# double125/MADTP

Measured on AMD Instinct MI355X. Metric: images/sec forward, BLIP-base NLVR2 p=0.5 b64; pruned-token index match, higher is better.
Workload: dtype bf16

## Files before the change

### madtp_amd/csrc/prune.hip

```cpp
#include "common.h"
#include "internal.h"
#include <stdlib.h>
#include <string.h>
#include <atomic>
#include <chrono>
#include <mutex>
#include <vector>

#ifndef TRY
#define TRY(x) do { int _rc = (x); if (_rc) return _rc; } while (0)
#endif

namespace {

constexpr int MAXN = 1024;

__device__ __forceinline__ float block_sum(float v, float* red, int tid, int nwaves) {
    v = wave_sum(v);
    __syncthreads();
    if ((tid & 63) == 0) red[tid >> 6] = v;
    __syncthreads();
    float s = 0.f;
    for (int w = 0; w < nwaves; ++w) s += red[w];
    return s;
// ... 1515 lines not shown
                for (int kk = 0; kk < 2; ++kk) {
                    ah[kk] = pack_bf16x8(xa[t][kk][0], xa[t][kk][1]);
                    f32x4 r0, r1;
#pragma unroll
                    for (int e = 0; e < 4; ++e) {
                        r0[e] = xa[t][kk][0][e] - bf16_to_f32((bf16_t)ah[kk][e]);
                        r1[e] = xa[t][kk][1][e] - bf16_to_f32((bf16_t)ah[kk][4 + e]);
                    }
                    al[kk] = pack_bf16x8(r0, r1);
                }
#pragma unroll
                for (int kk = 0; kk < 2; ++kk) {
#pragma unroll
                    for (int j = 0; j < 4; ++j) acc[t][j] = __builtin_amdgcn_mfma_f32_16x16x32_bf16(bh[kk][j], ah[kk], acc[t][j], 0, 0, 0);
#pragma unroll
                    for (int j = 0; j < 4; ++j) acc[t][j] = __builtin_amdgcn_mfma_f32_16x16x32_bf16(bh[kk][j], al[kk], acc[t][j], 0, 0, 0);
#pragma unroll
                    for (int j = 0; j < 4; ++j) acc[t][j] = __builtin_amdgcn_mfma_f32_16x16x32_bf16(bl[kk][j], ah[kk], acc[t][j], 0, 0, 0);
                }
            }
        }
    }
#pragma unroll
    for (int t = 0; t < 2; ++t) {
        const int m = row0 + rg * 32 + t * 16 + l16;
        if (m < M) {
            float* o = out + (size_t)m * 128 + cw * 64 + 4 * g;
#pragma unroll
            for (int j = 0; j < 4; ++j) *(f32x4*)(o + 16 * j) = F16 ? acc[t][j] * out_scale : acc[t][j];
        }
    }
}

}

constexpr int SPLIT_MAX_B = 1024, SPLIT_MAX_G = 8;
static std::atomic<int> g_score_fast{0};
static bool score_fast() { return g_score_fast.load(std::memory_order_relaxed) != 0; }
extern "C" int madtp_set_score_fast(int on) { return g_score_fast.exchange(on ? 1 : 0, std::memory_order_relaxed); }

static bool split_enabled() {
    static int v = -1;
    if (v < 0) { const char* e = getenv("MADTP_TS_SPLIT"); v = e ? atoi(e) : 1; }
    return v != 0;
}

static int token_score_launch(const float* colsum_part, int n_row_tiles, const float* p0, const float* onorm,
                              const float* token_attn, int ldt, int ldb, int K, float temperature, float* score,
                              float* threshold, int32_t* count, int32_t* kmax, int B, int H, int N, int32_t* done_ctr,
                              int32_t* host_slot, int seq, void* stream, int32_t* tick = nullptr, float* part = nullptr) {
    if (!colsum_part || !p0 || !onorm || !token_attn || !score || !threshold || !count) return MADTP_E_BADARG;
    if (B <= 0 || H <= 0 || N < 2 || n_row_tiles <= 0 || !(temperature > 0.f)) return MADTP_E_BADARG;
    if (N - 1 > MAXN || K > 128 || K <= 0 || ldt < K) return MADTP_E_SHAPE;
    const size_t stage_bytes = (size_t)(N - 1) * K * sizeof(float);
    const bool staged = K % 4 == 0 && ldt % 4 == 0 && ldb % 4 == 0 && aligned16(token_attn) && stage_bytes <= 140 * 1024;
    if (staged) {
        if (score_fast()) {
            MADTP_ENSURE_MAX_LDS((token_score_kernel<true, true>), 140 * 1024);
            hipLaunchKernelGGL((token_score_kernel<true, true>), dim3(B), dim3(512), stage_bytes, (hipStream_t)stream, colsum_part,
                               n_row_tiles, p0, onorm, token_attn, ldt, ldb, K, temperature, score, threshold, count, kmax, H, N,
                               done_ctr, host_slot, seq);
        } else {
            MADTP_ENSURE_MAX_LDS(token_score_kernel<true>, 140 * 1024);
            hipLaunchKernelGGL(token_score_kernel<true>, dim3(B), dim3(512), stage_bytes, (hipStream_t)stream, colsum_part,
                               n_row_tiles, p0, onorm, token_attn, ldt, ldb, K, temperature, score, threshold, count, kmax, H, N,
                               done_ctr, host_slot, seq);
// ... 357 lines not shown
        if (split) {
            MADTP_ENSURE_MAX_LDS(query_att_ft_mma_kernel<true>, att_ft_mma_lds(true));
            hipLaunchKernelGGL(att_ft_stats_kernel<true>, dim3(a.nseg, B), dim3(256), 0, (hipStream_t)stream, a, K, inv_sqrt_sd, stats);
            hipLaunchKernelGGL(query_att_ft_mma_kernel<true>, dim3(dim / AB_COLS, B), dim3(256), att_ft_mma_lds(true),
                               (hipStream_t)stream, a, K, stats, out, inv_sqrt_sd, acc_flag, dim);
        } else {
            MADTP_ENSURE_MAX_LDS(query_att_ft_mma_kernel<false>, att_ft_mma_lds(false));
            hipLaunchKernelGGL(att_ft_stats_kernel<false>, dim3(a.nseg, B), dim3(256), 0, (hipStream_t)stream, a, K, inv_sqrt_sd, stats);
            hipLaunchKernelGGL(query_att_ft_mma_kernel<false>, dim3(dim / AB_COLS, B), dim3(256), att_ft_mma_lds(false),
                               (hipStream_t)stream, a, K, stats, out, inv_sqrt_sd, acc_flag, dim);
        }
        MADTP_LAUNCH_CHECK();
    }
    return 0;
}

extern "C" int madtp_vector_gather(const float* vectors, const int64_t* indices, float* out, int B, int L, int K, int D,
                                   void* stream) {
    if (!vectors || !indices || !out || B <= 0 || L <= 0 || K <= 0 || D <= 0) return MADTP_E_BADARG;
    if (D % 4) return MADTP_E_SHAPE;
    if (!aligned16(vectors) || !aligned16(out)) return MADTP_E_ALIGN;
    const int rows = B * K;
    hipLaunchKernelGGL(vector_gather_kernel, dim3((rows + 3) / 4), dim3(256), 0, (hipStream_t)stream, vectors, indices, out, L,
                       K, D / 4, rows);
    MADTP_LAUNCH_CHECK();
    return 0;
}

extern "C" int madtp_align_logits(const float* x, const void* sd_hi, const void* sd_lo, float* out, int M, int dim,
                                  int split_dtype, float out_scale, void* stream) {
    return madtp_i_align_logits(x, sd_hi, sd_lo, out, M, dim, split_dtype, out_scale, DevN{nullptr, 0, 0}, stream);
}
static int align_rows_auto(int M) { (void)M; return 64; }

int madtp_i_align_logits(const float* x, const void* sd_hi, const void* sd_lo, float* out, int M, int dim, int split_dtype,
                         float out_scale, DevN m_dev, void* stream) {
    if (!x || !sd_hi || !sd_lo || !out || M <= 0) return MADTP_E_BADARG;
    if (split_dtype != MADTP_BF16 && split_dtype != MADTP_F16S) return MADTP_E_DTYPE;
    if (dim % 128) return MADTP_E_SHAPE;
    if (!aligned16(x) || !aligned16(sd_hi) || !aligned16(sd_lo) || !aligned16(out)) return MADTP_E_ALIGN;
    constexpr int lds = AL_STAGES * 2 * AL_TILE;
    MADTP_ENSURE_MAX_LDS(align_logits_kernel<12>, lds);
    MADTP_ENSURE_MAX_LDS(align_logits_kernel<8>, lds);
    MADTP_ENSURE_MAX_LDS(align_logits_kernel<0>, lds);
    static int variant = -1;
    if (variant < 0) { const char* e = getenv("MADTP_ALIGN_KERNEL"); variant = e ? atoi(e) : 0; }
    static int rows_env = -1;
    if (rows_env < 0) { const char* e = getenv("MADTP_ALIGN_ROWS"); rows_env = e ? atoi(e) : 0; }
    const int rows_sel = rows_env == 64 || rows_env == 128 ? rows_env : align_rows_auto(M);
    if ((variant == 0 || split_dtype == MADTP_F16S) && rows_sel == 128 && !m_dev.p) {
        MADTP_ENSURE_MAX_LDS(align_ws2_kernel<false>, 2 * AW2_STAGE);
        MADTP_ENSURE_MAX_LDS(align_ws2_kernel<true>, 2 * AW2_STAGE);
        if (split_dtype == MADTP_F16S)
            hipLaunchKernelGGL(align_ws2_kernel<true>, dim3((M + 127) / 128), dim3(768), 2 * AW2_STAGE, (hipStream_t)stream, x,
                               (const char*)sd_hi, (const char*)sd_lo, out, M, dim, out_scale, m_dev);
        else
            hipLaunchKernelGGL(align_ws2_kernel<false>, dim3((M + 127) / 128), dim3(768), 2 * AW2_STAGE, (hipStream_t)stream, x,
                               (const char*)sd_hi, (const char*)sd_lo, out, M, dim, 1.f, m_dev);
        MADTP_LAUNCH_CHECK();
        return 0;
    }
    if (variant == 0 || split_dtype == MADTP_F16S) {
        MADTP_ENSURE_MAX_LDS(align_ws_kernel<false>, 3 * AW_STAGE);
        MADTP_ENSURE_MAX_LDS(align_ws_kernel<true>, 3 * AW_STAGE);
        if (split_dtype == MADTP_F16S)
            hipLaunchKernelGGL(align_ws_kernel<true>, dim3((M + 63) / 64), dim3(768), 3 * AW_STAGE, (hipStream_t)stream, x,
                               (const char*)sd_hi, (const char*)sd_lo, out, M, dim, out_scale, m_dev);
        else
            hipLaunchKernelGGL(align_ws_kernel<false>, dim3((M + 63) / 64), dim3(768), 3 * AW_STAGE, (hipStream_t)stream, x,
                               (const char*)sd_hi, (const char*)sd_lo, out, M, dim, 1.f, m_dev);
        MADTP_LAUNCH_CHECK();
        return 0;
    }
    auto kern = dim == 768 ? align_logits_kernel<12> : dim == 512 ? align_logits_kernel<8> : align_logits_kernel<0>;
    hipLaunchKernelGGL(kern, dim3((M + 63) / 64), dim3(256), lds, (hipStream_t)stream, x, (const char*)sd_hi,
                       (const char*)sd_lo, out, M, dim, m_dev);
    MADTP_LAUNCH_CHECK();
    return 0;
}
```

### madtp_amd/csrc/gemm_device.h

```cpp
#pragma once
#include "common.h"
#include <type_traits>

namespace {


constexpr int ROWB = 128;
constexpr int NTHREADS = 256;

struct GemmArgs {
    const char* A; const char* W; const float* bias; const float* residual; void* C;
    int M, N, K, lda, ldw, ldc, ldr, act, ntm, ntn, dbg, fast_epi, splitk, ngrp;
    const char* A2; const char* W2; const float* bias2; void* C2; int pair;
    float out_scale;
    float acc_scale;
    float acc_scale2;
    float* sk_ws; int* sk_tick; int sk;
    int desc;
    int* range_flag;
    const int32_t* m_dev; int m_mul;
};
struct F16P { unsigned short bits; };

struct F16S {};
// ... 137 lines not shown
            for (int i = 0; i < 2; ++i) {
                const int row = min(row_t + 32 * i + l32, g.M - 1);
#pragma unroll
                for (int jv = 0; jv < NJ; ++jv)
                    rv[i][jv] = *(const f32x4*)(g.residual + (size_t)row * g.ldr + (cok[jv] ? colv[jv] : 0));
            }
        }
        __builtin_amdgcn_sched_barrier(0);
        __builtin_amdgcn_s_waitcnt(0x0F70);
        __builtin_amdgcn_sched_barrier(0);
#pragma unroll
        for (int i = 0; i < 2; ++i)
#pragma unroll
            for (int jv = 0; jv < NJ; ++jv) {
                const int t0 = LP_OUT ? 8 * jv : 4 * jv;
                f32x4 v[NV];
#pragma unroll
                for (int u = 0; u < NV; ++u) {
#pragma unroll
                    for (int e = 0; e < 4; ++e)
                        v[u][e] = epi_act<FAST_ACT, ACT>(fmaf(acc[i][j][t0 + 4 * u + e], g.acc_scale, bv[jv][u][e])) * g.out_scale;
                    if constexpr (HAS_RES) v[u] += rv[i][jv];
                }
                const unsigned off = cok[jv] ? (unsigned)((32 * i + l32) * ldc + colv[jv]) * CSZ : 0x80000000u;
                u32x4 bits;
                if constexpr (OM == OM_BF16) bits = __builtin_bit_cast(u32x4, pack_bf16x8(v[0], v[1]));
                else if constexpr (OM == OM_F16) bits = __builtin_bit_cast(u32x4, pack_f16x8(v[0], v[1]));
                else bits = __builtin_bit_cast(u32x4, v[0]);
                __builtin_amdgcn_raw_buffer_store_b128(bits, crsrc, off, 0, 0);
            }
    }
}

template <int OM, int ACT, bool HAS_RES, int FM, int FN, int BM, int BN, bool FAST_ONLY = false, int RM = 1, int RN = 1>
__device__ __forceinline__ void epilogue(const GemmArgs& g, const f32x4 (&acc)[FM][FN], const f32x4 (&res)[RM][RN],
                                         int m0, int n0, int wr, int wc, int l16, int grp4, size_t c_off) {
    constexpr bool LP_OUT = OM != OM_F32;
    constexpr bool FAST_ACT = OM == OM_BF16 || OM == OM_F16;
    const bool c_bf16 = g.ldc < 0;
    const int ldc = c_bf16 ? -g.ldc : g.ldc;
            const int col_w = n0 + wc * (BN / 2);
            if (FAST_ONLY || g.fast_epi) {
                constexpr int NJ = LP_OUT ? FN / 2 : FN;
                constexpr int NV = LP_OUT ? 2 : 1;
                constexpr int CSZ = LP_OUT ? 2 : 4;
                constexpr bool RES_PREF = !LP_OUT && RM == FM;
                float range_mx = 0.f;
                const int row_t = m0 + wr * (BM / 2);
                const int rows_valid = max(min(g.M - row_t, BM / 2), 0);
                const unsigned long long cb = (unsigned long long)((char*)g.C + (c_off + (size_t)((g.dbg & 8) ? (row_t & 127) : row_t) * ldc) * CSZ);
                const unsigned cb_lo = __builtin_amdgcn_readfirstlane((unsigned)cb);
                const unsigned cb_hi = __builtin_amdgcn_readfirstlane((unsigned)(cb >> 32));
                const __amdgpu_buffer_rsrc_t crsrc = __builtin_amdgcn_make_buffer_rsrc(
                    (void*)(((unsigned long long)cb_hi << 32) | cb_lo), 0,
                    __builtin_amdgcn_readfirstlane(rows_valid * ldc * CSZ), 0x00020000);
                int colv[NJ];
                bool cok[NJ];
                f32x4 bv[NJ][NV];
#pragma unroll
                for (int jv = 0; jv < NJ; ++jv) {
                    colv[jv] = col_w + (LP_OUT ? 32 * jv + 8 * grp4 : 16 * jv + 4 * grp4);
                    cok[jv] = colv[jv] < g.N;
#pragma unroll
                    for (int u = 0; u < NV; ++u) bv[jv][u] = (f32x4){0.f, 0.f, 0.f, 0.f};
                }
                if (g.bias) {
#pragma unroll
                    for (int jv = 0; jv < NJ; ++jv)
#pragma unroll
                        for (int u = 0; u < NV; ++u) bv[jv][u] = *(const f32x4*)(g.bias + (cok[jv] ? colv[jv] : 0) + 4 * u);
                }
                constexpr bool RES_LOAD = HAS_RES && !RES_PREF;
                constexpr int IC = RES_LOAD ? (FM > 2 ? FM / 2 : FM) : FM;
                f32x4 rv[RES_LOAD ? IC : 1][RES_LOAD ? NJ : 1][NV];
#pragma unroll
                for (int i0 = 0; i0 < FM; i0 += IC) {
                    if constexpr (RES_LOAD) {
#pragma unroll
                        for (int ii = 0; ii < IC; ++ii) {
                            const int row = min(row_t + l16 + 16 * (i0 + ii), g.M - 1);
#pragma unroll
                            for (int jv = 0; jv < NJ; ++jv) {
                                const float* rp = g.residual + (size_t)row * g.ldr + (cok[jv] ? colv[jv] : 0);
#pragma unroll
                                for (int u = 0; u < NV; ++u) rv[ii][jv][u] = *(const f32x4*)(rp + 4 * u);
                            }
                        }
                    }
                    if (RES_LOAD || i0 == 0) {
                        __builtin_amdgcn_sched_barrier(0);
                        __builtin_amdgcn_s_waitcnt(0x0F70);
                        __builtin_amdgcn_sched_barrier(0);
                    }
#pragma unroll
                    for (int ii = 0; ii < IC; ++ii) {
                        const int i = i0 + ii;
#pragma unroll
                        for (int jv = 0; jv < NJ; ++jv) {
                            f32x4 v[NV];
#pragma unroll
                            for (int u = 0; u < NV; ++u) {
#pragma unroll
                                for (int e = 0; e < 4; ++e)
                                    v[u][e] = epi_act<FAST_ACT, ACT>(fmaf(acc[i][NV * jv + u][e], g.acc_scale, bv[jv][u][e])) * g.out_scale;
                                if constexpr (RES_PREF && HAS_RES) v[u] += res[i][jv];
                                if constexpr (RES_LOAD) v[u] += rv[ii][jv][u];
                            }
                            const unsigned off = cok[jv] ? (unsigned)((16 * i + l16) * ldc + colv[jv]) * CSZ : 0x80000000u;
                            u32x4 bits;
                            if constexpr (OM == OM_F16S) {
                                u32x4 lo_bits;
                                split_f16x8(v[0], v[1], bits, lo_bits);
                                __builtin_amdgcn_raw_buffer_store_b128(lo_bits, crsrc, cok[jv] ? off + (unsigned)g.N * 2u : off, 0, 0);
                                range_mx = f16_range_acc(f16_range_acc(range_mx, v[0]), v[1]);
                            } else if constexpr (OM == OM_BF16) bits = __builtin_bit_cast(u32x4, pack_bf16x8(v[0], v[1]));
                            else if constexpr (OM == OM_F16) {
                                bits = __builtin_bit_cast(u32x4, pack_f16x8(v[0], v[1]));
                            }
                            else bits = __builtin_bit_cast(u32x4, v[0]);
                            __builtin_amdgcn_raw_buffer_store_b128(bits, crsrc, off, 0, 0);
                        }
                    }
                }
                if constexpr (OM == OM_F16S) f16_range_raise(g.range_flag, !(range_mx < 65520.0f));
            } else if constexpr (!FAST_ONLY) {
#pragma unroll
                for (int j = 0; j < FN; ++j)
#pragma unroll
                    for (int r = 0; r < 4; ++r) {
                        const int col = col_w + wfrag_row<LP_OUT>(j, 4 * grp4 + r);
                        if (col >= g.N) continue;
                        const float bv = g.bias ? g.bias[col] : 0.0f;
#pragma unroll
                        for (int i = 0; i < FM; ++i) {
                            const int row = m0 + wr * (BM / 2) + i * 16 + l16;
                            if (row >= g.M) continue;
                            float v = epi_act<FAST_ACT, ACT>(fmaf(acc[i][j][r], g.acc_scale, bv)) * g.out_scale;
                            if (g.residual) v += g.residual[(size_t)row * g.ldr + col];
                            const size_t ci = c_off + (size_t)row * ldc + col;
                            if constexpr (OM == OM_F16S) {
                                const _Float16 h = (_Float16)v;
                                ((_Float16*)g.C)[ci] = h;
                                ((_Float16*)g.C)[ci + g.N] = (_Float16)((v - (float)h) * F16S_LO_SCALE);
                                f16_range_raise(g.range_flag, f16_range_bad(v));
                            } else if constexpr (OM == OM_F16) {
                                ((_Float16*)g.C)[ci] = (_Float16)v;
                                f16_range_raise(g.range_flag, f16_range_bad(v));
                            } else if (c_bf16) ((bf16_t*)g.C)[ci] = f32_to_bf16(v);
                            else ((float*)g.C)[ci] = v;
                        }
                    }
            }
}

// ... 2 lines not shown
```

### madtp_amd/csrc/gemm_pp.hip

```cpp
#include "gemm_device.h"
#include <stdlib.h>

template <int OM, int MODE, int FA = 4, int ABL = 0, bool SPLITK = false>
__global__ __launch_bounds__(512, 2) void gemm_pp_kernel(GemmArgs g) {
    static_assert(FA == 4 || FA == 3, "256- or 192-row tiles");
    constexpr bool X3 = MODE == 2, F16 = MODE != 0;
    constexpr bool LP_OUT = OM != OM_F32;
    constexpr int BM = 64 * FA, BN = 256, HT = 128 * ROWB;
    extern __shared__ __attribute__((aligned(16))) char smem[];

    const int xcd = blockIdx.x & 7, lb = blockIdx.x >> 3, gl = gridDim.x >> 3;
    const int S = SPLITK ? g.splitk : 1;
    int t0, nslots;
    xcd_tiles(g.ntm * g.ntn * S, xcd, t0, nslots);
    if (lb >= nslots) return;

    const int tid = threadIdx.x, lane = tid & 63;
    const int wave = __builtin_amdgcn_readfirstlane(tid >> 6);
    const int wr = wave >> 2, wc = wave & 3;
    const int nkp = g.K / 64;
    const int nks = __builtin_amdgcn_readfirstlane(nkp / S);

    constexpr int WJ1 = (wfrag_row<LP_OUT>(1, 0) - wfrag_row<LP_OUT>(0, 0)) * ROWB;
    const char* ab[2][2];
    const char* wb[2][2];
    auto frag_bases = [&]() {
        int ln = lane;
        asm volatile("" : "+v"(ln));
        const int l16 = ln & 15, grp4 = ln >> 4;
        const int ra0 = wr * 64 + l16, rw0 = wc * 32 + wfrag_row<LP_OUT>(0, l16);
        const int a_rd = ra0 * ROWB + ((grp4 ^ (l16 & 7)) << 4);
        const int w_rd = rw0 * ROWB + ((grp4 ^ swz_key<LP_OUT>(rw0)) << 4);
        ab[0][0] = smem + a_rd; ab[0][1] = smem + (a_rd ^ 64); ab[1][0] = smem + 65536 + a_rd; ab[1][1] = smem + 65536 + (a_rd ^ 64);
        wb[0][0] = smem + w_rd; wb[0][1] = smem + (w_rd ^ 64); wb[1][0] = smem + 65536 + w_rd; wb[1][1] = smem + 65536 + (w_rd ^ 64);
    };
    frag_bases();

    const int npad = ((g.N + 127) / 128) * 128;
    const __amdgpu_buffer_rsrc_t rs_a = __builtin_amdgcn_make_buffer_rsrc((void*)g.A, 0, (unsigned)((size_t)g.M * g.lda * 2), 0x00020000);
    const __amdgpu_buffer_rsrc_t rs_w = __builtin_amdgcn_make_buffer_rsrc((void*)g.W, 0, (unsigned)((size_t)npad * g.ldw * 2), 0x00020000);
    unsigned va[2][2], vw[2][2];
    int is_slot = lb, is_koff = 0, is_kend = nkp * ROWB;
// ... 47 lines not shown
            is_koff += ROWB;                                                                   \
            if (is_koff == is_kend) { is_slot += gl; tile_offsets(); unit_krange(); }          \
        }                                                                                      \
        is_offa = is_koff + ((X3 && is_s == 2) ? plane_b : 0);                                 \
        is_offw = is_koff + ((X3 && is_s == 0) ? plane_b : 0);                                 \
    } while (0)

    f32x4 acc[2 * FA][4];
    bf16x8 a0[FA][2], a1[FA][2], b0[2][2], b1[2][2];
    const f32x4 zero4 = (f32x4){0.f, 0.f, 0.f, 0.f};
    f32x4 res[1][1];
#define PP_FENCE() __builtin_amdgcn_sched_barrier(0)
#define PP_READ_A(R, P, IDX)                                                                   \
    if (!(ABL & 4) || !steady)                                                                 \
    _Pragma("unroll") for (int i = 0; i < FA; ++i) {                                           \
        R[i][0] = *(const bf16x8*)(ab[P][0] + (IDX) * HT + i * 16 * ROWB);                     \
        R[i][1] = *(const bf16x8*)(ab[P][1] + (IDX) * HT + i * 16 * ROWB);                     \
    }
#define PP_READ_W(R, P, IDX)                                                                   \
    if (!(ABL & 4) || !steady)                                                                 \
    _Pragma("unroll") for (int j = 0; j < 2; ++j) {                                            \
        R[j][0] = *(const bf16x8*)(wb[P][0] + (IDX) * HT + j * WJ1);                           \
        R[j][1] = *(const bf16x8*)(wb[P][1] + (IDX) * HT + j * WJ1);                           \
    }
#define PP_MFMA(RA, RW, SA, SB)                                                                \
    if (!(ABL & 2))                                                                            \
    _Pragma("unroll") for (int ks = 0; ks < 2; ++ks)                                           \
        _Pragma("unroll") for (int i = 0; i < FA; ++i)                                         \
            _Pragma("unroll") for (int j = 0; j < 2; ++j)                                      \
                acc[(SA) * FA + i][(SB) * 2 + j] = mfma_16x16x32<F16>(RW[j][ks], RA[i][ks], acc[(SA) * FA + i][(SB) * 2 + j]);
#define PP_SCALE_W(R, ON)                                                                      \
    if constexpr (X3 && (ON))                                                                  \
    _Pragma("unroll") for (int j = 0; j < 2; ++j) { R[j][0] = x3_scale_lo(R[j][0]); R[j][1] = x3_scale_lo(R[j][1]); }
#define PP_PHASE(READS, ISSUE, PRE, MFMAS)                                                     \
    {                                                                                          \
        READS                                                                                  \
        PP_FENCE();                                                                            \
        if constexpr (!(ABL & 8)) { ISSUE }                                                    \
        PP_FENCE();                                                                            \
        wait_vmcnt<(ABL & 8) ? 8 : 10>();                                                      \
        PP_FENCE();                                                                            \
        __builtin_amdgcn_s_barrier();                                                          \
        PP_FENCE();                                                                            \
        if constexpr ((ABL & 8) != 0) { ISSUE }                                                \
        PP_FENCE();                                                                            \
        __builtin_amdgcn_s_waitcnt(0xC07F);                                    \
        PP_FENCE();                                                                            \
        PRE                                                                                    \
        PP_FENCE();                                                                            \
        if constexpr (!(ABL & 16)) __builtin_amdgcn_s_setprio(1);                              \
        MFMAS                                                                                  \
        if constexpr (!(ABL & 16)) __builtin_amdgcn_s_setprio(0);                              \
        PP_FENCE();                                                                            \
        __builtin_amdgcn_s_barrier();                                                          \
        PP_FENCE();                                                                            \
    }
#define PP_SLAB(P, SC)                                                                                                              \
    PP_PHASE(PP_READ_A(a0, P, 1), PP_ISSUE_W(vw[1], 4 * ((P) ^ 1) + 3); PP_NEXT_SLAB();, PP_SCALE_W(b0, SC), PP_MFMA(a0, b0, 0, 0))   \
    PP_PHASE(PP_READ_A(a1, P, 2), PP_ISSUE_W(vw[0], 4 * (P) + 0);, , PP_MFMA(a1, b0, 1, 0))                                          \
    PP_PHASE(PP_READ_W(b1, P, 3), PP_ISSUE_A(va[0], 4 * (P) + 1);, PP_SCALE_W(b1, SC), PP_MFMA(a1, b1, 1, 1))                        \
    PP_PHASE(PP_READ_W(b0, (P) ^ 1, 0), PP_ISSUE_A(va[1], 4 * (P) + 2);, , PP_MFMA(a0, b1, 0, 1))

    PP_ISSUE_W(vw[0], 0); PP_ISSUE_A(va[0], 1); PP_ISSUE_A(va[1], 2); PP_ISSUE_W(vw[1], 3);
    PP_NEXT_SLAB();
    PP_ISSUE_W(vw[0], 4); PP_ISSUE_A(va[0], 5); PP_ISSUE_A(va[1], 6);
    PP_FENCE();
    wait_vmcnt<10>();
    __builtin_amdgcn_s_barrier();
    PP_FENCE();

    for (int slot = lb; slot < nslots; slot += gl) {
        if (wr == 1) __builtin_amdgcn_s_barrier();
        PP_FENCE();
        if (slot != lb) { frag_bases(); tile_offsets(); }
        PP_READ_W(b0, 0, 0)
        PP_FENCE();
        __builtin_amdgcn_s_waitcnt(0xC07F);
        PP_FENCE();
#pragma unroll
        for (int i = 0; i < 2 * FA; ++i)
#pragma unroll
            for (int j = 0; j < 4; ++j) acc[i][j] = zero4;
        for (int kt = 0; kt < nks; kt += 2) {
            if constexpr (X3) {
                PP_SLAB(0, false)
                PP_SLAB(1, false)
                PP_SLAB(0, true)
                PP_SLAB(1, false)
                PP_SLAB(0, false)
                PP_SLAB(1, true)
            } else {
                PP_SLAB(0, false)
                PP_SLAB(1, false)
            }
            steady = true;
        }
        if (wr == 0) __builtin_amdgcn_s_barrier();
        PP_FENCE();
        int ctm, ctn;
        const int cu = t0 + slot, ct = S > 1 ? __builtin_amdgcn_readfirstlane(cu / S) : cu;
        tile_mn(g, ct, ctm, ctn);
        const size_t c_off = S > 1 ? (size_t)(cu - ct * S) * g.M * (size_t)(g.ldc < 0 ? -g.ldc : g.ldc) : 0;
        const int m0 = ctm * BM, n0 = ctn * BN + (wc >> 1) * 128;
        int lne = lane;
        asm volatile("" : "+v"(lne));
        const int l16e = lne & 15, grp4e = lne >> 4;
#define EPI(ACT)                                                                                                  \
    if constexpr (LP_OUT) {                                                                                       \
        epilogue<OM, ACT, false, 2 * FA, 4, BM, 128>(g, acc, res, m0, n0, wr, wc & 1, l16e, grp4e, c_off);             \
    } else {                                                                                                      \
        if (g.residual) epilogue<OM, ACT, true, 2 * FA, 4, BM, 128>(g, acc, res, m0, n0, wr, wc & 1, l16e, grp4e, c_off); \
        else epilogue<OM, ACT, false, 2 * FA, 4, BM, 128>(g, acc, res, m0, n0, wr, wc & 1, l16e, grp4e, c_off);        \
    }
        switch (g.act) {
            case MADTP_ACT_GELU_ERF: EPI(MADTP_ACT_GELU_ERF) break;
            case MADTP_ACT_QUICK_GELU: EPI(MADTP_ACT_QUICK_GELU) break;
            case MADTP_ACT_RELU: EPI(MADTP_ACT_RELU) break;
            default: EPI(MADTP_ACT_NONE) break;
        }
#undef EPI
    }
    wait_vmcnt<0>();
#undef PP_SLAB
#undef PP_PHASE
#undef PP_SCALE_W
#undef PP_ISSUE_A
#undef PP_ISSUE_W
#undef PP_MFMA
#undef PP_READ_W
#undef PP_READ_A
#undef PP_FENCE
#undef PP_NEXT_SLAB
#undef PP_ISSUE
}

__attribute__((visibility("hidden"))) int madtp_gemm_pp_launch(const void* args, int om, int mode, int rows, int grid, void* stream) {
    const GemmArgs& g = *(const GemmArgs*)args;
    hipStream_t s = (hipStream_t)stream;
    const size_t lds = (size_t)8 * 128 * ROWB;
    static int abl = -1;
    if (abl < 0) { const char* e = getenv("MADTP_PP_ABLATE"); abl = e ? atoi(e) : 0; }
#define PP_LAUNCH(OM_, MODE_, FA_, ABL_)                                                                        \
    do {                                                                                                        \
        MADTP_ENSURE_MAX_LDS((gemm_pp_kernel<OM_, MODE_, FA_, ABL_>), lds);                                      \
        hipLaunchKernelGGL((gemm_pp_kernel<OM_, MODE_, FA_, ABL_>), dim3(grid), dim3(512), lds, s, g);           \
    } while (0)
#define PP_ROWS(OM_, MODE_)                                                                                     \
    do { if (rows == 192) PP_LAUNCH(OM_, MODE_, 3, 0); else PP_LAUNCH(OM_, MODE_, 4, 0); } while (0)
    if (rows != 256 && rows != 192) return MADTP_E_BADARG;
    if (g.splitk > 1) {
        if (mode != 2 || om != OM_F32 || rows != 256 || g.bias || g.residual || g.act != MADTP_ACT_NONE) return MADTP_E_DTYPE;
        MADTP_ENSURE_MAX_LDS((gemm_pp_kernel<OM_F32, 2, 4, 0, true>), lds);
        hipLaunchKernelGGL((gemm_pp_kernel<OM_F32, 2, 4, 0, true>), dim3(grid), dim3(512), lds, s, g);
        return 0;
    }
    if (mode == 2) {
        if (om == OM_F16S) PP_ROWS(OM_F16S, 2); else if (om == OM_F32) PP_ROWS(OM_F32, 2); else return MADTP_E_DTYPE;
    } else if (mode == 1) {
        if (om == OM_F16) PP_ROWS(OM_F16, 1); else if (om == OM_F32) PP_ROWS(OM_F32, 1); else return MADTP_E_DTYPE;
    } else if (om == OM_BF16) {
        switch (rows == 256 ? abl : 0) {
#ifdef MADTP_PP_ABLATIONS
            case 1: PP_LAUNCH(OM_BF16, 0, 4, 1); break;
            case 2: PP_LAUNCH(OM_BF16, 0, 4, 2); break;
            case 3: PP_LAUNCH(OM_BF16, 0, 4, 3); break;
            case 4: PP_LAUNCH(OM_BF16, 0, 4, 4); break;
            case 5: PP_LAUNCH(OM_BF16, 0, 4, 5); break;
            case 6: PP_LAUNCH(OM_BF16, 0, 4, 6); break;
            case 8: PP_LAUNCH(OM_BF16, 0, 4, 8); break;
            case 16: PP_LAUNCH(OM_BF16, 0, 4, 16); break;
#endif
            default: PP_ROWS(OM_BF16, 0); break;
        }
    } else if (om == OM_F32) {
        PP_ROWS(OM_F32, 0);
    } else {
        return MADTP_E_DTYPE;
    }
#undef PP_ROWS
#undef PP_LAUNCH
    return 0;
}
```

Baseline: 26390.

## Add warp-specialized register-prefetch align-logits kernel with column split for small M

```diff
diff --git a/madtp_amd/csrc/prune.hip b/madtp_amd/csrc/prune.hip
--- a/madtp_amd/csrc/prune.hip
+++ b/madtp_amd/csrc/prune.hip
@@ -1571,6 +1571,147 @@
     }
 }
 
+constexpr int AR_STAGES = 4, AR_AHEAD = 3;
+template <bool F16, int NK, int COLS>
+__global__ __launch_bounds__(COLS * 6, 1) void align_rx_kernel(const float* __restrict__ x, const char* __restrict__ sd_hi,
+                                                               const char* __restrict__ sd_lo, float* __restrict__ out, int M,
+                                                               float out_scale, DevN m_dev) {
+    extern __shared__ __attribute__((aligned(16))) char smem[];
+    M = devn(m_dev, M);
+    if ((int)blockIdx.x * 64 >= M) return;
+    static_assert(COLS == 128 || COLS == 64, "column tile");
+    constexpr int dim = NK * 64;
+    constexpr int TILE = COLS * AL_ROWB, STAGE = 2 * TILE;
+    constexpr int NCONS = COLS / 16, PER = 8;
+    const int tid = threadIdx.x, lane = tid & 63;
+    const int wave = __builtin_amdgcn_readfirstlane(tid >> 6);
+    const int row0 = blockIdx.x * 64;
+    const int cb = COLS == 128 ? 0 : blockIdx.y * 64;
+    if (wave >= NCONS) {
+        const int lw = wave - NCONS;
+        const char* srcp[PER];
+#pragma unroll
+        for (int q = 0; q < PER; ++q) {
+            const int idx = lw * PER + q;
+            const int grp = idx % (COLS / 8), r = grp * 8 + (lane >> 3);
+            const char* base = idx < COLS / 8 ? sd_hi : sd_lo;
+            srcp[q] = base + (size_t)(cb + r) * dim * 2 + (((lane & 7) ^ (r & 7)) << 4);
+        }
+        auto issue = [&](int kt) {
+            char* st = smem + (kt % AR_STAGES) * STAGE + lw * PER * 1024;
+#pragma unroll
+            for (int q = 0; q < PER; ++q)
+                __builtin_amdgcn_global_load_lds(GLOBAL_PTR(srcp[q] + kt * AL_ROWB), LDS_PTR(st + q * 1024), 16, 0, 0);
+        };
+#pragma unroll
+        for (int kt = 0; kt < AR_AHEAD && kt < NK; ++kt) issue(kt);
+        for (int kt = 0; kt < NK; ++kt) {
+            if (kt + 2 < NK) asm volatile("s_waitcnt vmcnt(16)" ::: "memory");
+            else if (kt + 1 < NK) asm volatile("s_waitcnt vmcnt(8)" ::: "memory");
+            else asm volatile("s_waitcnt vmcnt(0)" ::: "memory");
+            __builtin_amdgcn_s_barrier();
+            if (kt + AR_AHEAD < NK) issue(kt + AR_AHEAD);
+        }
+        return;
+    }
+    const int l16 = lane & 15, g = lane >> 4;
+    const int rw = wave & 3, cw = wave >> 2;
+    const int xr = rw * 16 + l16;
+    const int cl = cw * 64;
+    int row = row0 + xr;
+    row = row < M ? row : M - 1;
+    const float* xp = x + (size_t)row * dim + g * 8;
+    f32x4 xq[AR_AHEAD][2][2];
+    auto load_x = [&](int kt, f32x4 (&d)[2][2]) {
+#pragma unroll
+        for (int kk = 0; kk < 2; ++kk) {
+            const float* p = xp + kt * 64 + kk * 32;
+            d[kk][0] = *(const f32x4*)p;
+            d[kk][1] = *(const f32x4*)(p + 4);
+        }
+    };
+#pragma unroll
+    for (int kt = 0; kt < AR_AHEAD && kt < NK; ++kt) load_x(kt, xq[kt]);
+    f32x4 acc[4];
+#pragma unroll
+    for (int j = 0; j < 4; ++j) acc[j] = (f32x4){0.f, 0.f, 0.f, 0.f};
+#pragma unroll
+    for (int kt = 0; kt < NK; ++kt) {
+        f32x4 (&xa)[2][2] = xq[kt % AR_AHEAD];
+        bf16x8 ah[2], al[2];
+        if constexpr (F16) {
+#pragma unroll
+            for (int kk = 0; kk < 2; ++kk) {
+                u32x4 p0, p1;
+                split_f16x8(xa[kk][0], xa[kk][1], p0, p1);
+                ah[kk] = __builtin_bit_cast(bf16x8, p0);
+                al[kk] = __builtin_bit_cast(bf16x8, p1);
+            }
+        } else {
+#pragma unroll
+            for (int kk = 0; kk < 2; ++kk) {
+                ah[kk] = pack_bf16x8(xa[kk][0], xa[kk][1]);
+                f32x4 r0, r1;
+#pragma unroll
+                for (int e = 0; e < 4; ++e) {
+                    r0[e] = xa[kk][0][e] - bf16_to_f32((bf16_t)ah[kk][e]);
+                    r1[e] = xa[kk][1][e] - bf16_to_f32((bf16_t)ah[kk][4 + e]);
+                }
+                al[kk] = pack_bf16x8(r0, r1);
+            }
+        }
+        __builtin_amdgcn_sched_barrier(0);
+        if (kt + AR_AHEAD < NK) load_x(kt + AR_AHEAD, xa);
+        const char* sh = smem + (kt % AR_STAGES) * STAGE;
+        const char* sl = sh + TILE;
+        __builtin_amdgcn_s_barrier();
+        bf16x8 bh[2][4], bl[2][4];
+#pragma unroll
+        for (int kk = 0; kk < 2; ++kk)
+#pragma unroll
+            for (int j = 0; j < 4; ++j) {
+                const int rb = cl + j * 16 + l16;
+                const int off = rb * AL_ROWB + (((kk * 4 + g) ^ (rb & 7)) << 4);
+                bh[kk][j] = *(const bf16x8*)(sh + off);
+                bl[kk][j] = *(const bf16x8*)(sl + off);
+            }
+        if constexpr (F16) {
+#pragma unroll
+            for (int kk = 0; kk < 2; ++kk) {
+#pragma unroll
+                for (int j = 0; j < 4; ++j)
+                    acc[j] = __builtin_amdgcn_mfma_f32_16x16x32_f16(__builtin_bit_cast(f16x8, bl[kk][j]), __builtin_bit_cast(f16x8, ah[kk]), acc[j], 0, 0, 0);
+#pragma unroll
+                for (int j = 0; j < 4; ++j)
+                    acc[j] = __builtin_amdgcn_mfma_f32_16x16x32_f16(__builtin_bit_cast(f16x8, bh[kk][j]), __builtin_bit_cast(f16x8, ah[kk]), acc[j], 0, 0, 0);
+#pragma unroll
+                for (int j = 0; j < 4; ++j) {
+                    const f16x8 q2 = __builtin_bit_cast(f16x8, bh[kk][j]) * (_Float16)(1.0f / F16S_LO_SCALE);
+                    acc[j] = __builtin_amdgcn_mfma_f32_16x16x32_f16(q2, __builtin_bit_cast(f16x8, al[kk]), acc[j], 0, 0, 0);
+                }
+            }
+        } else {
+#pragma unroll
+            for (int kk = 0; kk < 2; ++kk) {
+#pragma unroll
+                for (int j = 0; j < 4; ++j) acc[j] = __builtin_amdgcn_mfma_f32_16x16x32_bf16(bh[kk][j], ah[kk], acc[j], 0, 0, 0);
+#pragma unroll
+                for (int j = 0; j < 4; ++j) acc[j] = __builtin_amdgcn_mfma_f32_16x16x32_bf16(bh[kk][j], al[kk], acc[j], 0, 0, 0);
+#pragma unroll
+                for (int j = 0; j < 4; ++j) acc[j] = __builtin_amdgcn_mfma_f32_16x16x32_bf16(bl[kk][j], ah[kk], acc[j], 0, 0, 0);
+            }
+        }
+        asm volatile("s_waitcnt lgkmcnt(0)" ::: "memory");
+        __builtin_amdgcn_sched_barrier(0);
+    }
+    const int m = row0 + xr;
+    if (m < M) {
+        float* o = out + (size_t)m * 128 + cb + cl + 4 * g;
+#pragma unroll
+        for (int j = 0; j < 4; ++j) *(f32x4*)(o + 16 * j) = F16 ? acc[j] * out_scale : acc[j];
+    }
+}
+
 }
 
 constexpr int SPLIT_MAX_B = 1024, SPLIT_MAX_G = 8;
@@ -1994,6 +2135,7 @@
     return madtp_i_align_logits(x, sd_hi, sd_lo, out, M, dim, split_dtype, out_scale, DevN{nullptr, 0, 0}, stream);
 }
 static int align_rows_auto(int M) { (void)M; return 64; }
+static int align_variant_auto(int M) { return M <= 1280 ? 2 : 0; }
 
 int madtp_i_align_logits(const float* x, const void* sd_hi, const void* sd_lo, float* out, int M, int dim, int split_dtype,
                          float out_scale, DevN m_dev, void* stream) {
@@ -2010,6 +2152,31 @@
     static int rows_env = -1;
     if (rows_env < 0) { const char* e = getenv("MADTP_ALIGN_ROWS"); rows_env = e ? atoi(e) : 0; }
     const int rows_sel = rows_env == 64 || rows_env == 128 ? rows_env : align_rows_auto(M);
+    static int rx_env = -2;
+    if (rx_env == -2) { const char* e = getenv("MADTP_ALIGN_VARIANT"); rx_env = e ? atoi(e) : -1; }
+    const bool rx_ok = dim == 768 || dim == 512;
+    int rx = rx_env >= 0 ? rx_env : (rows_env == 64 || rows_env == 128 || variant != 0) ? 0 : align_variant_auto(M);
+    if (rx < 0 || rx > 2 || !rx_ok) rx = 0;
+    if (rx) {
+#define ALIGN_RX_LAUNCH(F16_, NK_, COLS_, SCALE_)                                                                              \
+    do {                                                                                                                       \
+        constexpr int lds_rx = AR_STAGES * 2 * COLS_ * AL_ROWB;                                                                \
+        MADTP_ENSURE_MAX_LDS((align_rx_kernel<F16_, NK_, COLS_>), lds_rx);                                                     \
+        hipLaunchKernelGGL((align_rx_kernel<F16_, NK_, COLS_>), dim3((M + 63) / 64, 128 / COLS_), dim3(COLS_ * 6), lds_rx,     \
+                           (hipStream_t)stream, x, (const char*)sd_hi, (const char*)sd_lo, out, M, SCALE_, m_dev);             \
+    } while (0)
+        const bool f16 = split_dtype == MADTP_F16S;
+        if (rx == 1) {
+            if (dim == 768) { if (f16) ALIGN_RX_LAUNCH(true, 12, 128, out_scale); else ALIGN_RX_LAUNCH(false, 12, 128, 1.f); }
+            else { if (f16) ALIGN_RX_LAUNCH(true, 8, 128, out_scale); else ALIGN_RX_LAUNCH(false, 8, 128, 1.f); }
+        } else {
+            if (dim == 768) { if (f16) ALIGN_RX_LAUNCH(true, 12, 64, out_scale); else ALIGN_RX_LAUNCH(false, 12, 64, 1.f); }
+            else { if (f16) ALIGN_RX_LAUNCH(true, 8, 64, out_scale); else ALIGN_RX_LAUNCH(false, 8, 64, 1.f); }
+        }
+#undef ALIGN_RX_LAUNCH
+        MADTP_LAUNCH_CHECK();
+        return 0;
+    }
     if ((variant == 0 || split_dtype == MADTP_F16S) && rows_sel == 128 && !m_dev.p) {
         MADTP_ENSURE_MAX_LDS(align_ws2_kernel<false>, 2 * AW2_STAGE);
         MADTP_ENSURE_MAX_LDS(align_ws2_kernel<true>, 2 * AW2_STAGE);
```

New measurement: 26150. About the same (-0.9%).

## Prefetch bias into LDS and double-buffer residual loads in GEMM epilogue

Applied to the files above, without the earlier changes.

```diff
diff --git a/madtp_amd/csrc/gemm_device.h b/madtp_amd/csrc/gemm_device.h
--- a/madtp_amd/csrc/gemm_device.h
+++ b/madtp_amd/csrc/gemm_device.h
@@ -193,9 +193,9 @@
     }
 }
 
-template <int OM, int ACT, bool HAS_RES, int FM, int FN, int BM, int BN, bool FAST_ONLY = false, int RM = 1, int RN = 1>
+template <int OM, int ACT, bool HAS_RES, int FM, int FN, int BM, int BN, bool FAST_ONLY = false, int RM = 1, int RN = 1, int BND = 0>
 __device__ __forceinline__ void epilogue(const GemmArgs& g, const f32x4 (&acc)[FM][FN], const f32x4 (&res)[RM][RN],
-                                         int m0, int n0, int wr, int wc, int l16, int grp4, size_t c_off) {
+                                         int m0, int n0, int wr, int wc, int l16, int grp4, size_t c_off, const char* sbias = nullptr) {
     constexpr bool LP_OUT = OM != OM_F32;
     constexpr bool FAST_ACT = OM == OM_BF16 || OM == OM_F16;
     const bool c_bf16 = g.ldc < 0;
@@ -208,7 +208,7 @@
                 constexpr bool RES_PREF = !LP_OUT && RM == FM;
                 float range_mx = 0.f;
                 const int row_t = m0 + wr * (BM / 2);
-                const int rows_valid = max(min(g.M - row_t, BM / 2), 0);
+                const int rows_valid = max(min(BND ? __builtin_amdgcn_readfirstlane(g.M - row_t) : g.M - row_t, BM / 2), 0);
                 const unsigned long long cb = (unsigned long long)((char*)g.C + (c_off + (size_t)((g.dbg & 8) ? (row_t & 127) : row_t) * ldc) * CSZ);
                 const unsigned cb_lo = __builtin_amdgcn_readfirstlane((unsigned)cb);
                 const unsigned cb_hi = __builtin_amdgcn_readfirstlane((unsigned)(cb >> 32));
@@ -229,29 +229,49 @@
 #pragma unroll
                     for (int jv = 0; jv < NJ; ++jv)
 #pragma unroll
-                        for (int u = 0; u < NV; ++u) bv[jv][u] = *(const f32x4*)(g.bias + (cok[jv] ? colv[jv] : 0) + 4 * u);
+                        for (int u = 0; u < NV; ++u) {
+                            if constexpr (BND & 1) bv[jv][u] = *(const f32x4*)(sbias + (colv[jv] - n0 + 4 * u) * 4);
+                            else bv[jv][u] = *(const f32x4*)(g.bias + (cok[jv] ? colv[jv] : 0) + 4 * u);
+                        }
                 }
                 constexpr bool RES_LOAD = HAS_RES && !RES_PREF;
-                constexpr int IC = RES_LOAD ? (FM > 2 ? FM / 2 : FM) : FM;
-                f32x4 rv[RES_LOAD ? IC : 1][RES_LOAD ? NJ : 1][NV];
+                constexpr bool RES_PIPE = RES_LOAD && (BND & 2) != 0 && !LP_OUT && (FM % 2) == 0 && FM > 2;
+                constexpr int IC = RES_PIPE ? 2 : (RES_LOAD ? (FM > 2 ? FM / 2 : FM) : FM);
+                [[maybe_unused]] constexpr int PER = IC * NJ * NV;
+                f32x4 rv[RES_PIPE ? 2 : 1][RES_LOAD ? IC : 1][RES_LOAD ? NJ : 1][NV];
+                auto res_load = [&](int b, int i0) {
+#pragma unroll
+                    for (int ii = 0; ii < IC; ++ii) {
+                        const int row = min(row_t + l16 + 16 * (i0 + ii), g.M - 1);
+#pragma unroll
+                        for (int jv = 0; jv < NJ; ++jv) {
+                            const float* rp = g.residual + (size_t)row * g.ldr + (cok[jv] ? colv[jv] : 0);
+#pragma unroll
+                            for (int u = 0; u < NV; ++u) rv[b][ii][jv][u] = *(const f32x4*)(rp + 4 * u);
+                        }
+                    }
+                };
+                if constexpr (RES_PIPE) {
+                    res_load(0, 0);
+                    __builtin_amdgcn_sched_barrier(0);
+                    res_load(1, IC);
+                }
 #pragma unroll
                 for (int i0 = 0; i0 < FM; i0 += IC) {
-                    if constexpr (RES_LOAD) {
-#pragma unroll
-                        for (int ii = 0; ii < IC; ++ii) {
-                            const int row = min(row_t + l16 + 16 * (i0 + ii), g.M - 1);
-#pragma unroll
-                            for (int jv = 0; jv < NJ; ++jv) {
-                                const float* rp = g.residual + (size_t)row * g.ldr + (cok[jv] ? colv[jv] : 0);
-#pragma unroll
-                                for (int u = 0; u < NV; ++u) rv[ii][jv][u] = *(const f32x4*)(rp + 4 * u);
-                            }
-                        }
-                    }
-                    if (RES_LOAD || i0 == 0) {
+                    const int rb = RES_PIPE ? (i0 / IC) & 1 : 0;
+                    if constexpr (RES_PIPE) {
                         __builtin_amdgcn_sched_barrier(0);
-                        __builtin_amdgcn_s_waitcnt(0x0F70);
+                        if (i0 == 0) wait_vmcnt<PER>();
+                        else if (i0 + IC < FM) wait_vmcnt<2 * PER>();
+                        else wait_vmcnt<PER>();
                         __builtin_amdgcn_sched_barrier(0);
+                    } else {
+                        if constexpr (RES_LOAD) res_load(0, i0);
+                        if (RES_LOAD || (i0 == 0 && !(BND & 1))) {
+                            __builtin_amdgcn_sched_barrier(0);
+                            __builtin_amdgcn_s_waitcnt(0x0F70);
+                            __builtin_amdgcn_sched_barrier(0);
+                        }
                     }
 #pragma unroll
                     for (int ii = 0; ii < IC; ++ii) {
@@ -265,7 +285,7 @@
                                 for (int e = 0; e < 4; ++e)
                                     v[u][e] = epi_act<FAST_ACT, ACT>(fmaf(acc[i][NV * jv + u][e], g.acc_scale, bv[jv][u][e])) * g.out_scale;
                                 if constexpr (RES_PREF && HAS_RES) v[u] += res[i][jv];
-                                if constexpr (RES_LOAD) v[u] += rv[ii][jv][u];
+                                if constexpr (RES_LOAD) v[u] += rv[rb][ii][jv][u];
                             }
                             const unsigned off = cok[jv] ? (unsigned)((16 * i + l16) * ldc + colv[jv]) * CSZ : 0x80000000u;
                             u32x4 bits;
@@ -281,6 +301,10 @@
                             else bits = __builtin_bit_cast(u32x4, v[0]);
                             __builtin_amdgcn_raw_buffer_store_b128(bits, crsrc, off, 0, 0);
                         }
+                    }
+                    if constexpr (RES_PIPE) {
+                        __builtin_amdgcn_sched_barrier(0);
+                        if (i0 + 2 * IC < FM) res_load(rb, i0 + 2 * IC);
                     }
                 }
                 if constexpr (OM == OM_F16S) f16_range_raise(g.range_flag, !(range_mx < 65520.0f));
diff --git a/madtp_amd/csrc/gemm_pp.hip b/madtp_amd/csrc/gemm_pp.hip
--- a/madtp_amd/csrc/gemm_pp.hip
+++ b/madtp_amd/csrc/gemm_pp.hip
@@ -1,13 +1,32 @@
 #include "gemm_device.h"
 #include <stdlib.h>
 
-template <int OM, int MODE, int FA = 4, int ABL = 0, bool SPLITK = false>
+#ifndef MADTP_PP_BOUNDARY
+#if defined(MADTP_PP_TIMING) && MADTP_PP_TIMING == 1
+#define MADTP_PP_BOUNDARY 0
+#else
+#define MADTP_PP_BOUNDARY 3
+#endif
+#endif
+#ifdef MADTP_PP_TIMING
+__device__ long long g_pp_dbg[32];
+__device__ __forceinline__ long long pp_now() {
+    __builtin_amdgcn_sched_barrier(0);
+    __builtin_amdgcn_s_waitcnt(0xC07F);
+    const long long t = wall_clock64();
+    __builtin_amdgcn_sched_barrier(0);
+    return t;
+}
+#endif
+template <int OM, int MODE, int FA = 4, int ABL = 0, bool SPLITK = false, bool GEN = false>
 __global__ __launch_bounds__(512, 2) void gemm_pp_kernel(GemmArgs g) {
     static_assert(FA == 4 || FA == 3, "256- or 192-row tiles");
     constexpr bool X3 = MODE == 2, F16 = MODE != 0;
     constexpr bool LP_OUT = OM != OM_F32;
     constexpr int BM = 64 * FA, BN = 256, HT = 128 * ROWB;
+    constexpr int BND = SPLITK ? 0 : (MADTP_PP_BOUNDARY);
     extern __shared__ __attribute__((aligned(16))) char smem[];
+    char* const sbias = smem + 8 * HT;
 
     const int xcd = blockIdx.x & 7, lb = blockIdx.x >> 3, gl = gridDim.x >> 3;
     const int S = SPLITK ? g.splitk : 1;
@@ -121,13 +140,23 @@
 #define PP_SCALE_W(R, ON)                                                                      \
     if constexpr (X3 && (ON))                                                                  \
     _Pragma("unroll") for (int j = 0; j < 2; ++j) { R[j][0] = x3_scale_lo(R[j][0]); R[j][1] = x3_scale_lo(R[j][1]); }
-#define PP_PHASE(READS, ISSUE, PRE, MFMAS)                                                     \
+#ifdef MADTP_PP_TIMING
+#define PP_WAIT(PH)                                                                            \
+    if (ts_first) {                                                                            \
+        const long long t__ = pp_now();                                                        \
+        wait_vmcnt<10>();                                                                      \
+        ts_ph##PH += pp_now() - t__;                                                           \
+    } else wait_vmcnt<10>()
+#else
+#define PP_WAIT(PH) wait_vmcnt<(ABL & 8) ? 8 : 10>()
+#endif
+#define PP_PHASE(PH, READS, ISSUE, PRE, MFMAS)                                                 \
     {                                                                                          \
         READS                                                                                  \
         PP_FENCE();                                                                            \
         if constexpr (!(ABL & 8)) { ISSUE }                                                    \
         PP_FENCE();                                                                            \
-        wait_vmcnt<(ABL & 8) ? 8 : 10>();                                                      \
+        PP_WAIT(PH);                                                                           \
         PP_FENCE();                                                                            \
         __builtin_amdgcn_s_barrier();                                                          \
         PP_FENCE();                                                                            \
@@ -145,10 +174,10 @@
         PP_FENCE();                                                                            \
     }
 #define PP_SLAB(P, SC)                                                                                                              \
-    PP_PHASE(PP_READ_A(a0, P, 1), PP_ISSUE_W(vw[1], 4 * ((P) ^ 1) + 3); PP_NEXT_SLAB();, PP_SCALE_W(b0, SC), PP_MFMA(a0, b0, 0, 0))   \
-    PP_PHASE(PP_READ_A(a1, P, 2), PP_ISSUE_W(vw[0], 4 * (P) + 0);, , PP_MFMA(a1, b0, 1, 0))                                          \
-    PP_PHASE(PP_READ_W(b1, P, 3), PP_ISSUE_A(va[0], 4 * (P) + 1);, PP_SCALE_W(b1, SC), PP_MFMA(a1, b1, 1, 1))                        \
-    PP_PHASE(PP_READ_W(b0, (P) ^ 1, 0), PP_ISSUE_A(va[1], 4 * (P) + 2);, , PP_MFMA(a0, b1, 0, 1))
+    PP_PHASE(0, PP_READ_A(a0, P, 1), PP_ISSUE_W(vw[1], 4 * ((P) ^ 1) + 3); PP_NEXT_SLAB();, PP_SCALE_W(b0, SC), PP_MFMA(a0, b0, 0, 0))   \
+    PP_PHASE(1, PP_READ_A(a1, P, 2), PP_ISSUE_W(vw[0], 4 * (P) + 0);, , PP_MFMA(a1, b0, 1, 0))                                          \
+    PP_PHASE(2, PP_READ_W(b1, P, 3), PP_ISSUE_A(va[0], 4 * (P) + 1);, PP_SCALE_W(b1, SC), PP_MFMA(a1, b1, 1, 1))                        \
+    PP_PHASE(3, PP_READ_W(b0, (P) ^ 1, 0), PP_ISSUE_A(va[1], 4 * (P) + 2);, , PP_MFMA(a0, b1, 0, 1))
 
     PP_ISSUE_W(vw[0], 0); PP_ISSUE_A(va[0], 1); PP_ISSUE_A(va[1], 2); PP_ISSUE_W(vw[1], 3);
     PP_NEXT_SLAB();
@@ -158,9 +187,27 @@
     __builtin_amdgcn_s_barrier();
     PP_FENCE();
 
+#ifdef MADTP_PP_TIMING
+    const bool ts_on = blockIdx.x == 0 && wc == 0;
+    long long ts_main = 0, ts_entry = 0, ts_epi = 0, ts_ph0 = 0, ts_ph1 = 0, ts_ph2 = 0, ts_ph3 = 0, ts_tiles = 0, ts_after = 0;
+    const long long ts_start = ts_on ? pp_now() : 0;
+    bool ts_first = false;
+#endif
     for (int slot = lb; slot < nslots; slot += gl) {
         if (wr == 1) __builtin_amdgcn_s_barrier();
         PP_FENCE();
+        if constexpr ((BND & 1) != 0) {
+            if (wave == 4 && g.bias && g.fast_epi) {
+                int btm, btn;
+                tile_mn(g, t0 + slot, btm, btn);
+                const __amdgpu_buffer_rsrc_t rs_b = __builtin_amdgcn_make_buffer_rsrc((void*)g.bias, 0, (unsigned)g.N * 4u, 0x00020000);
+                __builtin_amdgcn_raw_ptr_buffer_load_lds(rs_b, LDS_PTR(sbias), 16, (unsigned)lane * 16u, btn * (BN * 4), 0, 0);
+            }
+            PP_FENCE();
+        }
+#ifdef MADTP_PP_TIMING
+        const long long ts_t0 = ts_on ? pp_now() : 0;
+#endif
         if (slot != lb) { frag_bases(); tile_offsets(); }
         PP_READ_W(b0, 0, 0)
         PP_FENCE();
@@ -171,8 +218,15 @@
 #pragma unroll
             for (int j = 0; j < 4; ++j) acc[i][j] = zero4;
         for (int kt = 0; kt < nks; kt += 2) {
+#ifdef MADTP_PP_TIMING
+            ts_first = ts_on && kt == 0 && slot != lb;
+#define PP_TS_FIRST_OFF() ts_first = false;
+#else
+#define PP_TS_FIRST_OFF()
+#endif
             if constexpr (X3) {
                 PP_SLAB(0, false)
+                PP_TS_FIRST_OFF()
                 PP_SLAB(1, false)
                 PP_SLAB(0, true)
                 PP_SLAB(1, false)
@@ -180,36 +234,58 @@
                 PP_SLAB(1, true)
             } else {
                 PP_SLAB(0, false)
+                PP_TS_FIRST_OFF()
                 PP_SLAB(1, false)
             }
             steady = true;
         }
         if (wr == 0) __builtin_amdgcn_s_barrier();
         PP_FENCE();
+#ifdef MADTP_PP_TIMING
+        long long ts_t1 = 0;
+        if (ts_on) {
+            ts_t1 = pp_now();
+            ts_main += ts_t1 - ts_t0;
+            if constexpr (!(BND & 1)) { wait_vmcnt<0>(); const long long t__ = pp_now(); ts_entry += t__ - ts_t1; ts_t1 = t__; }
+        }
+#endif
         int ctm, ctn;
         const int cu = t0 + slot, ct = S > 1 ? __builtin_amdgcn_readfirstlane(cu / S) : cu;
         tile_mn(g, ct, ctm, ctn);
         const size_t c_off = S > 1 ? (size_t)(cu - ct * S) * g.M * (size_t)(g.ldc < 0 ? -g.ldc : g.ldc) : 0;
         const int m0 = ctm * BM, n0 = ctn * BN + (wc >> 1) * 128;
-        int lne = lane;
-        asm volatile("" : "+v"(lne));
-        const int l16e = lne & 15, grp4e = lne >> 4;
+        const char* const sbw = sbias + (wc >> 1) * 512;
 #define EPI(ACT)                                                                                                  \
+    int lne = lane;                                                                                               \
+    asm volatile("" : "+v"(lne));                                                                                 \
+    const int l16e = lne & 15, grp4e = lne >> 4;                                                                  \
     if constexpr (LP_OUT) {                                                                                       \
-        epilogue<OM, ACT, false, 2 * FA, 4, BM, 128>(g, acc, res, m0, n0, wr, wc & 1, l16e, grp4e, c_off);             \
+        epilogue<OM, ACT, false, 2 * FA, 4, BM, 128, !GEN, 1, 1, BND>(g, acc, res, m0, n0, wr, wc & 1, l16e, grp4e, c_off, sbw);             \
     } else {                                                                                                      \
-        if (g.residual) epilogue<OM, ACT, true, 2 * FA, 4, BM, 128>(g, acc, res, m0, n0, wr, wc & 1, l16e, grp4e, c_off); \
-        else epilogue<OM, ACT, false, 2 * FA, 4, BM, 128>(g, acc, res, m0, n0, wr, wc & 1, l16e, grp4e, c_off);        \
+        if (g.residual) epilogue<OM, ACT, true, 2 * FA, 4, BM, 128, !GEN, 1, 1, BND>(g, acc, res, m0, n0, wr, wc & 1, l16e, grp4e, c_off, sbw); \
+        else epilogue<OM, ACT, false, 2 * FA, 4, BM, 128, !GEN, 1, 1, BND>(g, acc, res, m0, n0, wr, wc & 1, l16e, grp4e, c_off, sbw);        \
     }
         switch (g.act) {
-            case MADTP_ACT_GELU_ERF: EPI(MADTP_ACT_GELU_ERF) break;
-            case MADTP_ACT_QUICK_GELU: EPI(MADTP_ACT_QUICK_GELU) break;
-            case MADTP_ACT_RELU: EPI(MADTP_ACT_RELU) break;
-            default: EPI(MADTP_ACT_NONE) break;
+            case MADTP_ACT_GELU_ERF: { EPI(MADTP_ACT_GELU_ERF) } break;
+            case MADTP_ACT_QUICK_GELU: { EPI(MADTP_ACT_QUICK_GELU) } break;
+            case MADTP_ACT_RELU: { EPI(MADTP_ACT_RELU) } break;
+            default: { EPI(MADTP_ACT_NONE) } break;
         }
 #undef EPI
+#ifdef MADTP_PP_TIMING
+        if (ts_on) { ts_epi += pp_now() - ts_t1; ts_tiles += 1; ts_after += slot != lb; }
+#endif
     }
     wait_vmcnt<0>();
+#ifdef MADTP_PP_TIMING
+    if (ts_on && lane == 0) {
+        long long* d = g_pp_dbg + 16 * wr;
+        d[0] = ts_main; d[1] = ts_entry; d[2] = ts_epi; d[3] = ts_ph0; d[4] = ts_ph1; d[5] = ts_ph2; d[6] = ts_ph3;
+        d[7] = ts_tiles; d[8] = pp_now() - ts_start; d[9] = ts_after;
+    }
+#endif
+#undef PP_WAIT
+#undef PP_TS_FIRST_OFF
 #undef PP_SLAB
 #undef PP_PHASE
 #undef PP_SCALE_W
@@ -223,24 +299,35 @@
 #undef PP_ISSUE
 }
 
+template <int OM_, int MODE_, int FA_, int ABL_>
+static int pp_launch_one(const GemmArgs& g, int grid, size_t lds, hipStream_t s) {
+    if constexpr (OM_ != OM_F32 && !(OM_ == OM_F16S && FA_ == 4)) {
+        if (g.fast_epi) {
+            MADTP_ENSURE_MAX_LDS((gemm_pp_kernel<OM_, MODE_, FA_, ABL_, false, false>), lds);
+            hipLaunchKernelGGL((gemm_pp_kernel<OM_, MODE_, FA_, ABL_, false, false>), dim3(grid), dim3(512), lds, s, g);
+            return 0;
+        }
+    }
+    MADTP_ENSURE_MAX_LDS((gemm_pp_kernel<OM_, MODE_, FA_, ABL_, false, true>), lds);
+    hipLaunchKernelGGL((gemm_pp_kernel<OM_, MODE_, FA_, ABL_, false, true>), dim3(grid), dim3(512), lds, s, g);
+    return 0;
+}
+
 __attribute__((visibility("hidden"))) int madtp_gemm_pp_launch(const void* args, int om, int mode, int rows, int grid, void* stream) {
     const GemmArgs& g = *(const GemmArgs*)args;
     hipStream_t s = (hipStream_t)stream;
-    const size_t lds = (size_t)8 * 128 * ROWB;
+    const size_t lds = (size_t)8 * 128 * ROWB + 1024;
     static int abl = -1;
     if (abl < 0) { const char* e = getenv("MADTP_PP_ABLATE"); abl = e ? atoi(e) : 0; }
 #define PP_LAUNCH(OM_, MODE_, FA_, ABL_)                                                                        \
-    do {                                                                                                        \
-        MADTP_ENSURE_MAX_LDS((gemm_pp_kernel<OM_, MODE_, FA_, ABL_>), lds);                                      \
-        hipLaunchKernelGGL((gemm_pp_kernel<OM_, MODE_, FA_, ABL_>), dim3(grid), dim3(512), lds, s, g);           \
-    } while (0)
+    do { const int rc__ = pp_launch_one<OM_, MODE_, FA_, ABL_>(g, grid, lds, s); if (rc__) return rc__; } while (0)
 #define PP_ROWS(OM_, MODE_)                                                                                     \
     do { if (rows == 192) PP_LAUNCH(OM_, MODE_, 3, 0); else PP_LAUNCH(OM_, MODE_, 4, 0); } while (0)
     if (rows != 256 && rows != 192) return MADTP_E_BADARG;
     if (g.splitk > 1) {
         if (mode != 2 || om != OM_F32 || rows != 256 || g.bias || g.residual || g.act != MADTP_ACT_NONE) return MADTP_E_DTYPE;
-        MADTP_ENSURE_MAX_LDS((gemm_pp_kernel<OM_F32, 2, 4, 0, true>), lds);
-        hipLaunchKernelGGL((gemm_pp_kernel<OM_F32, 2, 4, 0, true>), dim3(grid), dim3(512), lds, s, g);
+        MADTP_ENSURE_MAX_LDS((gemm_pp_kernel<OM_F32, 2, 4, 0, true, true>), lds);
+        hipLaunchKernelGGL((gemm_pp_kernel<OM_F32, 2, 4, 0, true, true>), dim3(grid), dim3(512), lds, s, g);
         return 0;
     }
     if (mode == 2) {
@@ -270,3 +357,9 @@
 #undef PP_LAUNCH
     return 0;
 }
+
+#ifdef MADTP_PP_TIMING
+extern "C" int madtp_debug_read_pp_ts(long long* out) {
+    return (int)hipMemcpyFromSymbol(out, HIP_SYMBOL(g_pp_dbg), sizeof(long long) * 32);
+}
+#endif
```

Measured after the change: 26560 before, 26390 after. No clear change (-0.6%).
